# Linyou/Ced-NeRF

Hardware: AMD Instinct MI355X
Metric: samples_per_sec (render_image_test, 800x800 D-NeRF lego-shaped synthetic) (higher is better)
Workload: dtype f32 (MLP GEMMs: split-fp16 MFMA, 22-bit operands, fp32 accumulate)

## Files before the change

ced_nerf_amd/csrc/field.hip:

```cpp
#include <atomic>
#include <cstring>

#include "ced_common.hpp"
#include "field_args.hpp"
#include "field_kernel.hpp"

namespace ced {

std::atomic<int> g_field_spread_tiles{ 2 };
std::atomic<int> g_march_two_pass{ -1 };

int launch_field(const ced_field_desc *d, FieldArgs &A, void *stream)
{
    int rc = validate_hash(&d->hash, "field_forward");
    if (rc) return rc;
    if (d->hash.n_levels != 16) {
        set_error("field_forward: the fused kernel needs n_levels == 16 (got %d)", d->hash.n_levels);
        return CED_E_UNSUPPORTED;
    }
    CED_REQUIRE(d->time_mode >= 0 && d->time_mode <= 2, "field_forward: time_mode=%d", d->time_mode);
    CED_REQUIRE(d->packed_weights != nullptr, "field_forward: null packed_weights");
    CED_REQUIRE(d->mlp_precision >= CED_MLP_F32 && d->mlp_precision <= CED_MLP_F32_HEAD16X2, "field_forward: mlp_precision=%d",
                d->mlp_precision);
    CED_REQUIRE((int64_t)d->packed_floats == ced_packed_weight_words(d->use_div_offsets, d->time_mode, d->mlp_precision),
// ... 37 lines not shown
};

}

extern "C" int ced_set_option(const char *key, int value)
{
    CED_REQUIRE(key != nullptr, "set_option: null key");
    if (strcmp(key, "field_spread_tiles") == 0) {
        CED_REQUIRE(value >= 0 && value <= 2, "set_option: field_spread_tiles must be 0, 1 or 2 (field_tile_range)");
        ced::g_field_spread_tiles = value;
        return CED_OK;
    }
    if (strcmp(key, "march_two_pass") == 0) {
        CED_REQUIRE(value >= -1 && value <= 1, "set_option: march_two_pass must be -1 (automatic), 0 or 1");
        ced::g_march_two_pass = value;
        return CED_OK;
    }
    if (strcmp(key, "hash_grad_blocks") == 0) {
        CED_REQUIRE(value >= 0 && value <= (1 << 20), "set_option: hash_grad_blocks must be 0 (no cap) .. 2^20");
        ced::g_hash_grad_blocks = value;
        return CED_OK;
    }
    ced::set_error("set_option: unknown key '%s'", key);
    return CED_E_INVALID;
}

extern "C" int64_t ced_packed_weight_floats(int use_div_offsets, int time_mode)
{
    (void)use_div_offsets;
    return time_mode ? ced::Blob<true>::TOTAL : ced::Blob<false>::TOTAL;
// ... 81 lines not shown
```

ced_nerf_amd/csrc/field_args.hpp:

```cpp
#pragma once
#include <hip/hip_runtime.h>
#include <atomic>
#include <cstdint>

#include "../../include/cednerf_hip.h"
#include "ced_common.hpp"

namespace ced {

struct HashLevels {
    float scale[CED_MAX_LEVELS];
    uint32_t res[CED_MAX_LEVELS], offset[CED_MAX_LEVELS], size[CED_MAX_LEVELS], hashed[CED_MAX_LEVELS];
};

inline void fill_levels(HashLevels &lv, const ced_hash_desc &h)
{
    for (int l = 0; l < CED_MAX_LEVELS; ++l) {
        lv.scale[l] = h.scale[l]; lv.res[l] = h.res[l]; lv.offset[l] = h.offset[l];
        lv.size[l] = h.size[l]; lv.hashed[l] = h.hashed[l];
    }
}

inline int require_32bit_byte_offsets(const ced_hash_desc &h, const char *who)
{
// ... 14 lines not shown
            pairs = pairs && l + 1 < h.n_levels && (uint64_t)h.offset[l] + h.size[l] < h.total_entries;
        }
        const int dense = dense_modes ? (pairs ? 3 : 1) : 0;
        word |= (n_hashed == 0 ? dense : (n_hashed == 4 ? 2 : 0)) << (2 * i);
    }
    return word;
}

struct FieldArgs {
    int64_t n;
    const int64_t *n_dev;
    unsigned long long *stamp;
    const int64_t *base_dev;
    const float *pos, *t, *dir;
    const float *rays_o, *rays_d;
    const int64_t *ray_idx;
    const int32_t *ray_idx32;
    const float *t0, *t1, *timestamps;
    int rays_mode, t_per_ray, want_rgb;
    float *rgb, *sigma, *geo;
    float aabb[6];
    float moving_step;
    int use_div, time_mode;
    const void *weights;
    int table_dtype, temporal;
    int spread_tiles;
    int level_mode;
    int max_blocks;
    const void *table;
    HashLevels levels;
};

extern std::atomic<int> g_march_two_pass;
extern std::atomic<int> g_field_spread_tiles;
extern std::atomic<int> g_hash_grad_blocks;
constexpr int kFieldBlocksDefault = 256;

template <int NT, int THREADS, typename Kernel>
void launch_field_grid(Kernel kernel, const FieldArgs &A, void *stream)
{
    const int64_t n_tiles = (A.n + 16 * NT - 1) / (16 * NT);
    constexpr int waves = THREADS / 64;
    int64_t blocks = A.spread_tiles ? (n_tiles + 3) / 4 : (n_tiles + waves - 1) / waves;
    const int cap = A.max_blocks > 0 ? A.max_blocks : kFieldBlocksDefault;
    if (blocks > cap) blocks = cap;
    hipLaunchKernelGGL(kernel, dim3((unsigned)blocks), dim3(THREADS), 0, (hipStream_t)stream, A);
}

int validate_hash(const ced_hash_desc *h, const char *who);
// ... 6 lines not shown
```

ced_nerf_amd/csrc/field_device.hpp:

```cpp
#pragma once
#include <cstdint>

#include "ced_common.hpp"

namespace ced {

typedef float f4 __attribute__((ext_vector_type(4)));
typedef float f2 __attribute__((ext_vector_type(2)));

struct TileRange { int64_t first, end, stride; };
__device__ __forceinline__ bool field_tile_range(int mode, int64_t n_tiles, int waves, int wave, TileRange &r)
{
    const int64_t grid = gridDim.x, b = blockIdx.x;
    if (mode == 2 && (grid & 7) == 0) {
        const int64_t n_groups = (n_tiles + 3) >> 2, per_xcd = grid >> 3, region = (n_groups + 7) >> 3;
        const int64_t start = (b & 7) * region;
        const int64_t g_end = start + region < n_groups ? start + region : n_groups;
        if (start + (b >> 3) >= g_end) return false;
        r.first = (start + (int64_t)(wave >> 2) * per_xcd + (b >> 3)) * 4 + (wave & 3);
        r.end = 4 * g_end < n_tiles ? 4 * g_end : n_tiles;
        r.stride = (int64_t)(waves / 4) * per_xcd * 4;
        return true;
    }
    if ((mode ? b * 4 : b * waves) >= n_tiles) return false;
// ... 73 lines not shown
{
    typedef uint32_t u4 __attribute__((ext_vector_type(4)));
    const u4 a = *reinterpret_cast<const u4 *>(lt), b = *reinterpret_cast<const u4 *>(lt + 4);
    LevelConst L;
    L.scale = __uint_as_float(a[0]);
    L.sxb = a[1];
    L.syb = a[2];
    L.szb = a[3];
    L.offb = b[0];
    L.sizeb = b[1];
    L.maskb = b[2];
    L.hashed = b[3];
    return L;
}

template <bool F16, bool TEMPORAL, int MODE>
__device__ __forceinline__ void hash_level(const LevelConst &L, const void *__restrict__ table, const float (&x)[3],
                                           int k_lo, float t_frac, float &f0, float &f1)
{
    uint32_t g[3];
    float fr[3], om[3];
#pragma unroll
    for (int a = 0; a < 3; ++a) {
        const float p = x[a] * L.scale + 0.5f;
        g[a] = (uint32_t)p;
        fr[a] = __builtin_amdgcn_fractf(p);
        om[a] = 1.0f - fr[a];
    }
    constexpr uint32_t EB = EntryBytes<F16, TEMPORAL>::value;
    const uint32_t x0 = g[0] * EB;
    const uint32_t y0 = (MODE == 1 || MODE == 3) ? __umul24(g[1], L.syb) : g[1] * L.syb;
    const uint32_t z0 = (MODE == 1 || MODE == 3) ? __umul24(g[2], L.szb) : g[2] * L.szb;
    const uint32_t xs[2] = { x0, x0 + EB };
    const uint32_t ys[2] = { y0, y0 + L.syb };
    const uint32_t zs[2] = { z0, z0 + L.szb };
    const bool hashed = L.hashed != 0;
    uint32_t yz_x[4], yz_a[4];
#pragma unroll
    for (int q = 0; q < 4; ++q) {
        if constexpr (MODE != 1 && MODE != 3) yz_x[q] = ys[q & 1] ^ zs[q >> 1];
        if constexpr (MODE != 2) yz_a[q] = ys[q & 1] + zs[q >> 1];
    }
    const float wxy[4] = { om[0] * om[1], fr[0] * om[1], om[0] * fr[1], fr[0] * fr[1] };
    uint32_t off[8];
    float w[8];
#pragma unroll
    for (int c = 0; c < 8; ++c) {
        const int cx = c & 1, cy = (c >> 1) & 1, cz = (c >> 2) & 1;
        uint32_t hb = 0, db = 0;
        if constexpr (MODE != 1 && MODE != 3) hb = (xs[cx] ^ yz_x[cy + 2 * cz]) & L.maskb;
        if constexpr (MODE != 2) {
            const uint32_t dx = xs[cx] + yz_a[cy + 2 * cz];
            const uint32_t dw = dx - L.sizeb;
            db = dx < dw ? dx : dw;
        }
        const uint32_t idxb = (MODE == 1 || MODE == 3) ? db : (MODE == 2) ? hb : (hashed ? hb : db);
        off[c] = L.offb + idxb;
        w[c] = wxy[cx + 2 * cy] * (cz ? fr[2] : om[2]);
    }
    const char *tb = reinterpret_cast<const char *>(table);
    f2 v[8];
    if constexpr (!TEMPORAL) {
        if constexpr (MODE == 3) {
            constexpr uint32_t EBp = EntryBytes<F16, TEMPORAL>::value;
#pragma unroll
            for (int q = 0; q < 4; ++q) {
                if constexpr (!F16) {
                    const f4 pr = *reinterpret_cast<const f4 *>(tb + off[2 * q]);
                    v[2 * q] = f2{ pr[0], pr[1] };
                    v[2 * q + 1] = f2{ pr[2], pr[3] };
                    if (off[2 * q + 1] != off[2 * q] + EBp) v[2 * q + 1] = *reinterpret_cast<const f2 *>(tb + off[2 * q + 1]);
                } else {
                    typedef uint32_t u2v __attribute__((ext_vector_type(2)));
                    const u2v u = *reinterpret_cast<const u2v *>(tb + off[2 * q]);
                    uint32_t u1 = u[1];
                    if (off[2 * q + 1] != off[2 * q] + EBp) u1 = *reinterpret_cast<const uint32_t *>(tb + off[2 * q + 1]);
                    v[2 * q] = f2{ half_bits_to_float((uint16_t)(u[0] & 0xffffu)), half_bits_to_float((uint16_t)(u[0] >> 16)) };
                    v[2 * q + 1] = f2{ half_bits_to_float((uint16_t)(u1 & 0xffffu)), half_bits_to_float((uint16_t)(u1 >> 16)) };
                }
            }
        } else if constexpr (!F16) {
#pragma unroll
            for (int c = 0; c < 8; ++c) v[c] = *reinterpret_cast<const f2 *>(tb + off[c]);
        } else {
#pragma unroll
            for (int c = 0; c < 8; ++c) {
                const uint32_t u = *reinterpret_cast<const uint32_t *>(tb + off[c]);
                v[c] = f2{ half_bits_to_float((uint16_t)(u & 0xffffu)), half_bits_to_float((uint16_t)(u >> 16)) };
            }
        }
    } else {
        const float omt = 1.0f - t_frac;
        const f2 omt2 = { omt, omt }, tf2 = { t_frac, t_frac };
        const uint32_t kb = (uint32_t)k_lo * (F16 ? 4u : 8u);
        if constexpr (!F16) {
#pragma unroll
            for (int c = 0; c < 8; ++c) {
                const f4 pr = *reinterpret_cast<const f4 *>(tb + off[c] + kb);
                const f2 lo = { pr[0], pr[1] }, hi = { pr[2], pr[3] };
                v[c] = lo * omt2 + hi * tf2;
            }
        } else {
#pragma unroll
            for (int c = 0; c < 8; ++c) {
                typedef uint32_t u2t __attribute__((ext_vector_type(2)));
                const u2t pr = *reinterpret_cast<const u2t *>(tb + off[c] + kb);
                const uint32_t lo = pr[0], hi = pr[1];
                const f2 a = { half_bits_to_float((uint16_t)(lo & 0xffffu)), half_bits_to_float((uint16_t)(lo >> 16)) };
                const f2 b = { half_bits_to_float((uint16_t)(hi & 0xffffu)), half_bits_to_float((uint16_t)(hi >> 16)) };
                v[c] = a * omt2 + b * tf2;
            }
        }
    }
    f2 acc = { 0.0f, 0.0f };
#pragma unroll
    for (int c = 0; c < 8; ++c) acc = __builtin_elementwise_fma(f2{ w[c], w[c] }, v[c], acc);
    f0 = acc[0];
    f1 = acc[1];
}

template <bool F16, bool TEMPORAL, int MODE>
__device__ __forceinline__ void hash_level_dx(const LevelConst &L, const void *__restrict__ table, const float (&x)[3],
                                              int k_lo, float t_frac, float dscale, float &f0, float &f1, float (&d0)[3],
                                              float (&d1)[3])
{
    static_assert(MODE == 0 || MODE == 2, "hash_level_dx: mixed (0) or hashed (2) index form");
    uint32_t g[3];
// ... 59 lines not shown
    f2 gx = { 0.0f, 0.0f }, gy = { 0.0f, 0.0f }, gz = { 0.0f, 0.0f };
#pragma unroll
    for (int q = 0; q < 4; ++q) {
        const int lo = q & 1, hi = q >> 1;
        const float wyz = (lo ? fr[1] : om[1]) * (hi ? fr[2] : om[2]);
        const float wxz = (lo ? fr[0] : om[0]) * (hi ? fr[2] : om[2]);
        gx = __builtin_elementwise_fma(f2{ wyz, wyz }, v[1 + 2 * lo + 4 * hi] - v[2 * lo + 4 * hi], gx);
        gy = __builtin_elementwise_fma(f2{ wxz, wxz }, v[lo + 2 + 4 * hi] - v[lo + 4 * hi], gy);
        gz = __builtin_elementwise_fma(f2{ wxy[q], wxy[q] }, v[q + 4] - v[q], gz);
    }
    const float s = L.scale * dscale;
    d0[0] = gx[0] * s; d0[1] = gy[0] * s; d0[2] = gz[0] * s;
    d1[0] = gx[1] * s; d1[1] = gy[1] * s; d1[2] = gz[1] * s;
}

__device__ __forceinline__ void temporal_keyframe(float tq, int &k_lo, float &t_frac)
{
    float ts = tq * 3.0f;
    float fl = __builtin_floorf(ts);
    t_frac = ts - fl;
    fl = __builtin_fminf(fl, 2.0f);
    k_lo = (int)fl;
}

__device__ __forceinline__ float time_feature(int idx, int time_mode, float t, float mn)
{
    const float HALF_PI = 1.57079637050628662f;
    if (idx == 0) return t;
    if (idx > 8) return 0.0f;
    int k, ph;
// ... 14 lines not shown
```

ced_nerf_amd/csrc/field_half.hip:

```cpp
#include <cstring>

#include "ced_common.hpp"
#include "field_args.hpp"
#include "field_device.hpp"
#include "field_half_device.hpp"
#include "hash_device.hpp"

namespace ced {

template <bool TE, bool F16, bool TEMPORAL, bool SPLIT, int NT, int THREADS>
__global__ __launch_bounds__(THREADS) void field_half_kernel(FieldArgs A)
{
    constexpr int WAVES = THREADS / kWave;
    constexpr bool K32 = half_kernel_k32(TE, TEMPORAL, SPLIT, THREADS);
    static_assert(!K32 || (WAVES & (WAVES - 1)) == 0, "field_tile_seq needs a power-of-two wave count");
    constexpr int TILE = 16 * NT;
    using BL = HalfBlob<TE>;
    constexpr int PLANE = BL::FRAGS * kFragHalves;
    constexpr int WHALVES = PLANE * (SPLIT ? 2 : 1);
    __shared__ __attribute__((aligned(16))) _Float16 lds[WHALVES + 16 * CED_MAX_LEVELS];
    __shared__ int next_elem;
    const int tid = threadIdx.x;
    const int lane = tid & 63;
    const int wave = __builtin_amdgcn_readfirstlane(tid >> 6);
// ... 181 lines not shown
#pragma unroll
        for (int j = 0; j < NT; ++j) {
            const bool stored = 16 * j + c < in_tile;
            const int64_t s = tile_base + (16 * j + c);
            float sg = det_expf(D[j][0][3] - 1.0f);
            sg = sel[j] ? sg : 0.0f;
            if (g == 3 && stored) A.sigma[sbase + s] = sg;
            if (A.geo && stored) {
#pragma unroll
                for (int r = 0; r < 4; ++r)
                    if (4 * g + r < 15) A.geo[s * 15 + 4 * g + r] = D[j][0][r];
            }
        }

        if (A.want_rgb) {
#pragma unroll
            for (int j = 0; j < NT; ++j) {
                float dv[3];
#pragma unroll
                for (int a = 0; a < 3; ++a)
                    dv[a] = A.rays_mode ? A.rays_d[3 * ridx[j] + a] : A.dir[3 * (tile_base + sofs[j]) + a];
                const float nrm = __builtin_sqrtf((dv[0] * dv[0] + dv[1] * dv[1]) + dv[2] * dv[2]);
                const float comp = (g == 1) ? dv[1] : (g == 2) ? dv[2] : dv[0];
                const float u = (comp / nrm + 1.0f) / 2.0f;
                const float vv = u * 2.0f - 1.0f;
                const float coef = (g == 2) ? 0.48860251190291987f : -0.48860251190291987f;
                const float sh = (g == 0) ? 0.28209479177387814f : coef * vv;
                float hin[8];
                hin[0] = sh;
#pragma unroll
                for (int r = 0; r < 4; ++r) hin[1 + r] = __builtin_amdgcn_fmed3f(D[j][0][r], -kHalfMax, kHalfMax);
                hin[4] = (g == 3) ? 0.0f : hin[4];
                hin[5] = hin[6] = hin[7] = 0.0f;
                to_half8<SPLIT>(hin, Bh[j][0], Bl[j][0]);
            }
            mlp_layer_h<1, 4, NT, SPLIT>(whi + BL::H0 * kFragHalves, wlo + BL::H0 * kFragHalves, lane, Bh, Bl, D);
            to_operand_h<NT, SPLIT>(D, Bh, Bl);
            mlp_layer_h<2, 4, NT, SPLIT, K32>(whi + BL::H1 * kFragHalves, wlo + BL::H1 * kFragHalves, lane, Bh, Bl, D);
            to_operand_h<NT, SPLIT>(D, Bh, Bl);
            mlp_layer_h<2, 1, NT, SPLIT, K32>(whi + BL::H2 * kFragHalves, wlo + BL::H2 * kFragHalves, lane, Bh, Bl, D);
#pragma unroll
            for (int j = 0; j < NT; ++j) {
                const int64_t s = tile_base + (16 * j + c);
                const float o1 = 1.0f / (1.0f + det_expf(-D[j][0][0]));
// ... 142 lines not shown
```

ced_nerf_amd/csrc/field_kernel.hpp:

```cpp
#pragma once
#include "ced_common.hpp"
#include "field_args.hpp"
#include "field_device.hpp"
#include "field_half_device.hpp"
#include "hash_device.hpp"

namespace ced {

struct LayerShape { int nb; int ks; };
__host__ __device__ constexpr int ks4_of(int ks) { return (ks + 3) / 4; }
__host__ __device__ constexpr int layer_floats(int nb, int ks) { return nb * ks4_of(ks) * 256; }

__host__ __device__ constexpr int base_out_neuron(int p)
{
    const int g = p >> 2, r = p & 3;
    return r > 0 ? (4 * r + g - 3) : (g < 3 ? 13 + g : 0);
}

template <bool TE> struct Blob {
    static constexpr int KS_B0 = TE ? 11 : 8;
    static constexpr int M0 = 0;
    static constexpr int M1 = M0 + layer_floats(4, 8);
    static constexpr int M2 = M1 + layer_floats(4, 16);
    static constexpr int M3 = M2 + layer_floats(4, 16);
// ... 267 lines not shown
#pragma unroll
                for (int r = 0; r < 4; ++r) {
                    const int nidx = HEAD16 ? half_base_out_neuron(4 * g + r) : base_out_neuron(4 * g + r);
                    if (nidx >= 1) A.geo[s * 15 + nidx - 1] = D[j][0][r];
                }
            }
        }

        if constexpr (HEAD16) {
            if (A.want_rgb) {
                const _Float16 *const hw = reinterpret_cast<const _Float16 *>(lw + BL::H0);
                const _Float16 *const hwl = hw + BL::HEAD_FRAGS * kFragHalves;
                h8 Bh[NT][2], Bl[NT][2];
#pragma unroll
                for (int j = 0; j < NT; ++j) {
                    float dv[3];
#pragma unroll
                    for (int a = 0; a < 3; ++a)
                        dv[a] = A.rays_mode ? A.rays_d[3 * ridx[j] + a] : A.dir[3 * sidx[j] + a];
                    const float nrm = __builtin_sqrtf((dv[0] * dv[0] + dv[1] * dv[1]) + dv[2] * dv[2]);
                    const float comp = (g == 1) ? dv[1] : (g == 2) ? dv[2] : dv[0];
                    const float u = (comp / nrm + 1.0f) / 2.0f;
                    const float vv = u * 2.0f - 1.0f;
                    const float coef = (g == 2) ? 0.48860251190291987f : -0.48860251190291987f;
                    float hin[8];
                    hin[0] = (g == 0) ? 0.28209479177387814f : coef * vv;
#pragma unroll
                    for (int r = 0; r < 4; ++r) hin[1 + r] = __builtin_amdgcn_fmed3f(D[j][0][r], -kHalfMax, kHalfMax);
                    hin[4] = (g == 3) ? 0.0f : hin[4];
                    hin[5] = hin[6] = hin[7] = 0.0f;
                    to_half8<true>(hin, Bh[j][0], Bl[j][0]);
                }
                mlp_layer_h<1, 4, NT, true>(hw + BL::HF_H0 * kFragHalves, hwl + BL::HF_H0 * kFragHalves, lane, Bh, Bl, D);
                to_operand_h<NT, true>(D, Bh, Bl);
                mlp_layer_h<2, 4, NT, true>(hw + BL::HF_H1 * kFragHalves, hwl + BL::HF_H1 * kFragHalves, lane, Bh, Bl, D);
                to_operand_h<NT, true>(D, Bh, Bl);
                mlp_layer_h<2, 1, NT, true>(hw + BL::HF_H2 * kFragHalves, hwl + BL::HF_H2 * kFragHalves, lane, Bh, Bl, D);
#pragma unroll
                for (int j = 0; j < NT; ++j) {
                    const float o1 = 1.0f / (1.0f + det_expf(-D[j][0][0]));
                    int lane_now = (int)threadIdx.x;
                    asm volatile("" : "+v"(lane_now));
                    const int g_now = (lane_now >> 4) & 3;
                    const int64_t s_now = tile * TILE + 16 * j + (lane_now & 15);
                    if (g_now < 3 && s_now < n_eff) A.rgb[3 * (sbase + s_now) + g_now] = o1;
                }
            }
            continue;
        }

        if (A.want_rgb) {
#pragma unroll
            for (int j = 0; j < NT; ++j) {
                const float geo_tail = (g == 3) ? 0.0f : D[j][0][0];
                float dv[3];
#pragma unroll
                for (int a = 0; a < 3; ++a)
                    dv[a] = A.rays_mode ? A.rays_d[3 * ridx[j] + a] : A.dir[3 * sidx[j] + a];
                const float nrm = __builtin_sqrtf((dv[0] * dv[0] + dv[1] * dv[1]) + dv[2] * dv[2]);
                const float comp = (g == 1) ? dv[1] : (g == 2) ? dv[2] : dv[0];
                const float u = (comp / nrm + 1.0f) / 2.0f;
                const float vv = u * 2.0f - 1.0f;
                const float coef = (g == 2) ? 0.48860251190291987f : -0.48860251190291987f;
                B[j][0] = (g == 0) ? 0.28209479177387814f : coef * vv;
                B[j][1] = D[j][0][1];
                B[j][2] = D[j][0][2];
                B[j][3] = D[j][0][3];
                B[j][4] = geo_tail;
            }
            mlp_layer<5, 4, NT>(lw + BL::H0, lane, B, D);
            to_operand<4, true, NT>(D, B);
            mlp_layer<16, 4, NT>(lw + BL::H1, lane, B, D);
            to_operand<4, true, NT>(D, B);
            mlp_layer<16, 1, NT>(lw + BL::H2, lane, B, D);
#pragma unroll
            for (int j = 0; j < NT; ++j) {
                const int64_t s = tile * TILE + 16 * j + c;
                const float o1 = 1.0f / (1.0f + det_expf(-D[j][0][0]));
                int lane_now = (int)threadIdx.x;
// ... 12 lines not shown
```

ced_nerf_amd/csrc/frame.hip:

```cpp
#include <atomic>
#include <chrono>
#include <vector>

#include "ced_common.hpp"
#include "composite_core.hpp"
#include "field_args.hpp"
#include "march_accel.hpp"

#ifdef CED_MARCH_DIAG
__device__ unsigned long long g_march_diag[8][3];
__device__ __forceinline__ unsigned long long (*ced_diag_acc())[8][3]
{
    __shared__ unsigned long long acc[16][8][3];
    return acc;
}
__device__ __forceinline__ unsigned long long *ced_diag_state()
{
    __shared__ unsigned long long st[16][2];
    return &st[0][0];
}
__device__ void ced_diag_tick(int phase)
{
    const unsigned long long m = __ballot(1);
    const int wave = threadIdx.x >> 6;
// ... 129 lines not shown
    return block_base + wave_cnt[wave] + __builtin_popcountll(ballot & ((1ull << lane) - 1ull));
}

__global__ __launch_bounds__(256) void frame_times_kernel(int64_t n_rays, int rays_per_frame,
                                                          const float *__restrict__ frame_times, float *__restrict__ ts_ray)
{
    const int64_t r = (int64_t)blockIdx.x * blockDim.x + threadIdx.x;
    if (r < n_rays) ts_ray[r] = frame_times[r / rays_per_frame];
}

__global__ __launch_bounds__(256) void frame_prep_kernel(int64_t n_rays, const float *__restrict__ rays_o,
                                                         const float *__restrict__ rays_d, int m,
                                                         const float *__restrict__ aabbs, float near_plane,
                                                         float *__restrict__ t_sorted, uint8_t *__restrict__ t_indices,
                                                         uint8_t *__restrict__ hits, float *__restrict__ near_planes,
                                                         float *__restrict__ rgb,
                                                         float *__restrict__ opacity, float *__restrict__ depth)
{
    int64_t r = (int64_t)blockIdx.x * blockDim.x + threadIdx.x;
    if (r >= n_rays) return;
    const float o[3] = { rays_o[3 * r], rays_o[3 * r + 1], rays_o[3 * r + 2] };
    const float inv_d[3] = { 1.0f / rays_d[3 * r], 1.0f / rays_d[3 * r + 1], 1.0f / rays_d[3 * r + 2] };
    float ev[2 * kMaxGrids];
    int id[2 * kMaxGrids];
    for (int a = 0; a < m; ++a) {
        float t0 = __builtin_inff(), t1 = __builtin_inff();
        bool hit = slab_test(o, inv_d, aabbs + 6 * a, t0, t1);
        if (!hit) { t0 = __builtin_inff(); t1 = __builtin_inff(); }
        hits[r * m + a] = hit ? 1 : 0;
        ev[a] = t0; id[a] = a;
        ev[m + a] = t1; id[m + a] = m + a;
    }
    if (m > 1) {
        for (int i = 1; i < 2 * m; ++i) {
            float v = ev[i];
            int k = id[i], j = i - 1;
            while (j >= 0 && ev[j] > v) { ev[j + 1] = ev[j]; id[j + 1] = id[j]; --j; }
            ev[j + 1] = v; id[j + 1] = k;
        }
    }
    for (int i = 0; i < 2 * m; ++i) {
        t_sorted[r * 2 * m + i] = ev[i];
        t_indices[r * 2 * m + i] = (uint8_t)id[i];
    }
    near_planes[r] = near_plane;
    rgb[3 * r] = 0.0f; rgb[3 * r + 1] = 0.0f; rgb[3 * r + 2] = 0.0f;
    opacity[r] = 0.0f;
    depth[r] = 0.0f;
}

__global__ __launch_bounds__(256) void frame_prep_single_kernel(int64_t n_rays, float near_plane, float *__restrict__ near_planes,
                                                                float *__restrict__ rgb, float *__restrict__ opacity,
                                                                float *__restrict__ depth)
{
    int64_t r = (int64_t)blockIdx.x * blockDim.x + threadIdx.x;
    if (r >= n_rays) return;
    near_planes[r] = near_plane;
    rgb[3 * r] = 0.0f; rgb[3 * r + 1] = 0.0f; rgb[3 * r + 2] = 0.0f;
    opacity[r] = 0.0f;
    depth[r] = 0.0f;
}

struct ScheduleArgs {
    IterPlan *plans;
    int it, n_frames, rays_per_frame, min_samples, max_samples;
    long long *host;
    long long seq;
    const int32_t *local_rays;
    const int64_t *xcounts;
    int64_t global_rays;
    long long *host_iter;
// ... 319 lines not shown
{
    const int f = threadIdx.x;
    if (f >= n_frames) return;
    const unsigned long long nx = __hip_atomic_load(&plan->next[f], __ATOMIC_RELAXED, __HIP_MEMORY_SCOPE_AGENT);
    const bool finished = plan->last[f] || plan->gcount[f] == 0 || plan->count[f] == 0;
    row[f] = finished ? 0 : (int64_t)(nx & 0xffffffffull);
}

struct ImageState {
    int32_t *cursor;
    float *acc_all;
    float *acc_kept;
    int32_t *kept;
};

__global__ __launch_bounds__(256) void image_prep_kernel(int64_t n_rays, ImageState st, float *__restrict__ rgb,
                                                         float *__restrict__ opacity, float *__restrict__ depth)
{
    int64_t r = (int64_t)blockIdx.x * blockDim.x + threadIdx.x;
    if (r >= n_rays) return;
    st.cursor[r] = 0; st.acc_all[r] = 0.0f; st.acc_kept[r] = 0.0f; st.kept[r] = 0;
    if (rgb) {
        rgb[3 * r] = 0.0f; rgb[3 * r + 1] = 0.0f; rgb[3 * r + 2] = 0.0f;
        opacity[r] = 0.0f;
        depth[r] = 0.0f;
    }
}

__device__ __forceinline__ int64_t ray_count(const int64_t *__restrict__ packed_all, int64_t r, int64_t n_all)
{
    const int64_t start = packed_all[2 * r], cnt = packed_all[2 * r + 1];
    return (start < 0 || cnt < 0 || start + cnt > n_all) ? 0 : cnt;
}

__global__ __launch_bounds__(kMarchThreads) void image_chunk_kernel(
    IterPlan *__restrict__ plan, int64_t n_all, const int32_t *__restrict__ alive, const int64_t *__restrict__ packed_all,
    const float *__restrict__ t0_all, const float *__restrict__ t1_all, const int32_t *__restrict__ cursor,
// ... 220 lines not shown
    {
        T *p = (T *)(base + off);
        off = (off + count * sizeof(T) + 255) & ~(size_t)255;
        return p;
    }
};

struct FrameWorkspace {
    float *t_sorted; uint8_t *t_indices; uint8_t *hits; float *near; int32_t *packed;
    int32_t *alive_a, *alive_b;
    IterPlan *plans;
    float *lattice;
    float *ts_ray;
    float *t0, *t1; int32_t *ridx; float *sigma, *rgbs;
    uint8_t *accel;
    size_t bytes;
};

static inline int min_samples_of(float cone_angle) { return cone_angle == 0.0f ? 1 : 4; }
static inline int max_iterations(int max_samples, int min_samples) { return (max_samples + min_samples - 1) / min_samples; }

static inline int64_t sample_capacity(int n_frames, int64_t rays_per_frame, int min_samples, int64_t global_rays)
{
    int64_t per = rays_per_frame * min_samples;
    if (global_rays > rays_per_frame) {
        const int64_t worst = rays_per_frame * 64 < global_rays ? rays_per_frame * 64 : global_rays;
        if (worst > per) per = worst;
    }
    return per * n_frames;
}
// ... 7 lines not shown
    w.hits = c.take<uint8_t>((size_t)n * m);
    w.near = c.take<float>((size_t)n);
    w.packed = c.take<int32_t>((size_t)n * 2);
    w.alive_a = c.take<int32_t>((size_t)n);
    w.alive_b = c.take<int32_t>((size_t)n);
    w.plans = c.take<IterPlan>((size_t)max_iters + 2);
    w.lattice = c.take<float>(256);
    w.ts_ray = c.take<float>(per_ray_times ? (size_t)n : 0);
    w.t0 = c.take<float>((size_t)cap);
    w.t1 = c.take<float>((size_t)cap);
    w.ridx = c.take<int32_t>((size_t)cap);
    w.sigma = c.take<float>((size_t)cap);
    w.rgbs = c.take<float>((size_t)cap * 3);
    const int64_t nbk = (res + kBrick - 1) / kBrick;
    w.accel = c.take<uint8_t>((size_t)(2 * m * nbk * nbk * nbk));
    w.bytes = c.off;
    return w;
}

static std::atomic<long long> g_publish_seq{ 0 };

#if defined(__HIP_DEVICE_COMPILE__)
#define CED_CPU_PAUSE()
#else
#define CED_CPU_PAUSE() __builtin_ia32_pause()
#endif

static int wait_published(volatile long long *flag, long long seq, hipStream_t stream, const char *who)
{
    const auto t_start = std::chrono::steady_clock::now();
// ... 92 lines not shown
    CED_REQUIRE(cap < (1ll << 31) - 64, "%s: too many samples per iteration for 32-bit sample indices", who);
    const int max_iters = max_iterations(max_samples, min_samples);
    FrameWorkspace W = carve(workspace, n_rays, n_grids, cap, max_iters, res, frame_times != nullptr);
    CED_REQUIRE((int64_t)W.bytes <= workspace_bytes, "%s: workspace too small (%lld < %lld bytes)", who,
                (long long)workspace_bytes, (long long)W.bytes);
    if (xch) {
        CED_REQUIRE(xch->reduce && xch->counts && xch->global_rays_per_frame >= rays_per_frame &&
                        xch->global_rays_per_frame < (1ll << 31),
                    "%s: bad ced_shard_exchange (reduce / counts NULL, or global_rays_per_frame < rays_per_frame)", who);
        CED_REQUIRE(!field_stream_ || field_stream_ == stream_, "%s: a sharded call takes no separate field stream", who);
    }
    long long *const host_iter = xch ? (long long *)host_stats + kHostIterWord : nullptr;
    const dim3 blk(256), grd((unsigned)((n_rays + 255) / 256));

    if (n_grids == 1)
        hipLaunchKernelGGL(frame_prep_single_kernel, grd, blk, 0, stream, n_rays, near_plane, W.near, rgb, opacity, depth);
    else
        hipLaunchKernelGGL(frame_prep_kernel, grd, blk, 0, stream, n_rays, rays_o, rays_d, (int)n_grids, aabbs, near_plane,
                           W.t_sorted, W.t_indices, W.hits, W.near, rgb, opacity, depth);
    if (frame_times)
        hipLaunchKernelGGL(frame_times_kernel, grd, blk, 0, stream, n_rays, (int)rays_per_frame, frame_times, W.ts_ray);
    const int nb = (res + kBrick - 1) / kBrick;
    AccelSpec acc;
    if (accel) {
        acc = accel_view(accel, n_grids, res, true);
    } else {
        int rc = build_brick_accel(binaries, n_grids, res, W.accel, W.accel + (size_t)n_grids * nb * nb * nb, stream);
        if (rc) return rc;
        acc = AccelSpec{ W.accel, nb, nullptr };
    }
    volatile long long *pub = (volatile long long *)host_stats;
    std::vector<long long> plan_seq((size_t)max_iters + 1);
    plan_seq[0] = ++g_publish_seq;
    const bool use_lattice = cone_angle == 0.0f && step_size > 0.0f && near_plane >= 0.0f;
// ... 42 lines not shown
            }
        } else if (it == 0) {
            if (n_grids == 1) hipLaunchKernelGGL((march_frame_kernel<true, false, true>), dim3((unsigned)mgrid), mblk, 0, stream, M, plan);
            else hipLaunchKernelGGL((march_frame_kernel<false, false, true>), dim3((unsigned)mgrid), mblk, 0, stream, M, plan);
        } else {
            if (n_grids == 1) hipLaunchKernelGGL((march_frame_kernel<true, false, false>), dim3((unsigned)mgrid), mblk, 0, stream, M, plan);
            else hipLaunchKernelGGL((march_frame_kernel<false, false, false>), dim3((unsigned)mgrid), mblk, 0, stream, M, plan);
        }
        rc = check_launch("render_image_test (march)");
        if (rc) return rc;

        FieldArgs F{};
        F.n = cap;
        F.n_dev = &plan->total_samples;
        F.rays_o = rays_o; F.rays_d = rays_d; F.ray_idx32 = W.ridx;
        F.t0 = W.t0; F.t1 = W.t1;
        F.timestamps = frame_times ? W.ts_ray : timestamps;
        F.rays_mode = 1; F.t_per_ray = (frame_times || t_per_ray) ? 1 : 0; F.want_rgb = 1;
        F.rgb = W.rgbs; F.sigma = W.sigma; F.geo = nullptr;
        if (trace && trace->field_stamps && it < trace->capacity)
            F.stamp = reinterpret_cast<unsigned long long *>(trace->field_stamps) + 2 * it;
        if (split) {
            (void)hipEventRecord(ev_to_field[dev], stream);
            (void)hipStreamWaitEvent(fstream, ev_to_field[dev], 0);
        }
        if (trace && it < trace->capacity && trace->field_begin)
            (void)hipEventRecord((hipEvent_t)trace->field_begin[it], fstream);
        rc = launch_field(field, F, (void *)fstream);
        if (rc) return rc;
        if (trace && it < trace->capacity && trace->field_end)
// ... 52 lines not shown
            if (trace->iter_n_samples) trace->iter_n_samples[k] = max_limit;
            if (trace->iter_samples) trace->iter_samples[k] = samples_it;
        }
    }
    if (trace) trace->n_iters = n_iters;
    if (total_samples_out)
        for (int f = 0; f < n_frames; ++f) total_samples_out[f] = total[f];
    return CED_OK;
}

struct ImageWorkspace {
    ImageState st;
    int32_t *packed, *alive_a, *alive_b;
    IterPlan *plans;
    float *t0, *t1; int32_t *ridx; float *sigma, *rgbs, *w, *tr, *al; int32_t *rank;
    size_t bytes;
};

constexpr int kImageMaxIters = 1024;

static ImageWorkspace carve_image(void *base, int64_t n, int64_t cap)
{
    ImageWorkspace w{};
    Carver c{ (char *)base };
    w.st.cursor = c.take<int32_t>((size_t)n);
    w.st.acc_all = c.take<float>((size_t)n);
    w.st.acc_kept = c.take<float>((size_t)n);
    w.packed = c.take<int32_t>((size_t)n * 2);
    w.alive_a = c.take<int32_t>((size_t)n);
    w.alive_b = c.take<int32_t>((size_t)n);
    w.plans = c.take<IterPlan>((size_t)kImageMaxIters + 2);
    w.t0 = c.take<float>((size_t)cap);
    w.t1 = c.take<float>((size_t)cap);
    w.ridx = c.take<int32_t>((size_t)cap);
    w.sigma = c.take<float>((size_t)cap);
    w.rgbs = c.take<float>((size_t)cap * 3);
    w.w = c.take<float>((size_t)cap);
    w.tr = c.take<float>((size_t)cap);
    w.al = c.take<float>((size_t)cap);
    w.rank = c.take<int32_t>((size_t)cap);
    w.bytes = c.off;
    return w;
}

static inline int64_t image_capacity(int64_t n_rays, int64_t n_all) { return n_all + 64; }

static int render_image_impl(const ced_field_desc *field, int64_t n_rays, const float *rays_o, const float *rays_d,
                             int64_t n_all, const int64_t *packed_all, const float *t0_all, const float *t1_all,
                             float early_stop_eps, float alpha_thre, const float *timestamps, int32_t t_per_ray,
                             const float *bkgd, float *rgb, float *opacity, float *depth, int32_t *kept, void *workspace,
                             int64_t workspace_bytes, int64_t *host_stats, int64_t *stats_out, void *field_stream_,
                             void *stream_)
{
    const char *who = "render_image";
    hipStream_t stream = (hipStream_t)stream_;
// ... 2 lines not shown
    CED_REQUIRE(field != nullptr, "%s: null field descriptor", who);
    CED_REQUIRE(n_rays >= 0 && n_all >= 0, "%s: bad sizes", who);
    CED_REQUIRE(n_rays < (1ll << 31) / 4 && n_all < (1ll << 31) - 128, "%s: too many rays / samples for 32-bit indices", who);
    if (stats_out) { stats_out[0] = 0; stats_out[1] = 0; stats_out[2] = 0; }
    if (n_rays == 0) return CED_OK;
    const bool full = rgb != nullptr;
    CED_REQUIRE(rays_o && rays_d && packed_all && (n_all == 0 || (t0_all && t1_all)) && timestamps && kept && workspace &&
                    host_stats && (!full || (opacity && depth)),
                "%s: null pointer", who);
    const int64_t cap = image_capacity(n_rays, n_all);
    ImageWorkspace W = carve_image(workspace, n_rays, cap);
    W.st.kept = kept;
    CED_REQUIRE((int64_t)W.bytes <= workspace_bytes, "%s: workspace too small (%lld < %lld bytes)", who,
                (long long)workspace_bytes, (long long)W.bytes);
    const dim3 blk(256), grd((unsigned)((n_rays + 255) / 256));
    hipLaunchKernelGGL(image_prep_kernel, grd, blk, 0, stream, n_rays, W.st, rgb, opacity, depth);
    volatile long long *pub = (volatile long long *)host_stats;
    std::vector<long long> plan_seq((size_t)kImageMaxIters + 1);
    plan_seq[0] = ++g_publish_seq;
    const int big = 1 << 30;
    const int min_chunk = full ? 4 : 8;
    hipLaunchKernelGGL(frame_init_kernel, dim3(1), dim3(64), 0, stream,
                       ScheduleArgs{ W.plans, -1, 1, (int)n_rays, min_chunk, big, (long long *)host_stats, plan_seq[0] }, (float *)nullptr,
                       (unsigned long long *)nullptr, 0);
    int rc = check_launch("render_image (prep)");
    if (rc) return rc;
    long long alive_bound = n_rays;
    int it = 0;
    for (; it < kImageMaxIters; ++it) {
        bool stop = false;
        rc = run_ahead(pub, nullptr, plan_seq, it, stream, who, stop, alive_bound);
        if (rc) return rc;
        if (stop) break;
        IterPlan *plan = W.plans + it;
        const int32_t *cur_list = it == 0 ? nullptr : ((it & 1) ? W.alive_a : W.alive_b);
        int32_t *next_list = (it & 1) ? W.alive_b : W.alive_a;
        int64_t mgrid = (alive_bound + kMarchThreads - 1) / kMarchThreads;
        if (mgrid > 8192) mgrid = 8192;
        if (mgrid < 1) mgrid = 1;
        hipLaunchKernelGGL(image_chunk_kernel, dim3((unsigned)mgrid), dim3(kMarchThreads), 0, stream, plan, n_all, cur_list,
                           packed_all, t0_all, t1_all, W.st.cursor, W.t0, W.t1, W.ridx, W.packed);
        FieldArgs F{};
        F.n = n_rays * (int64_t)min_chunk;
        F.n_dev = &plan->total_samples;
        F.base_dev = &plan->sample_base;
        F.rays_o = rays_o; F.rays_d = rays_d; F.ray_idx32 = W.ridx;
        F.t0 = W.t0; F.t1 = W.t1;
        F.timestamps = timestamps;
        F.rays_mode = 1; F.t_per_ray = t_per_ray ? 1 : 0; F.want_rgb = full ? 1 : 0;
        F.rgb = full ? W.rgbs : nullptr; F.sigma = W.sigma; F.geo = nullptr;
        rc = launch_field(field, F, (void *)stream);
        if (rc) return rc;
        int64_t cgrid = (alive_bound + kCompositeThreads - 1) / kCompositeThreads;
        if (cgrid > 4096) cgrid = 4096;
        if (cgrid < 1) cgrid = 1;
        plan_seq[it + 1] = ++g_publish_seq;
        if (full)
            hipLaunchKernelGGL(image_composite_kernel<true>, dim3((unsigned)cgrid), dim3(kCompositeThreads), 0, stream, plan,
                               cur_list, next_list, W.packed, packed_all, W.t0, W.t1, W.sigma, W.rgbs, W.st, W.w, W.tr, W.al,
                               W.rank, rgb, opacity, depth, early_stop_eps, alpha_thre, n_all);
        else
// ... 202 lines not shown
```

Measured before the change: 4.471 billion.

## Precompute per-ray SH inputs and add dense-level fast path for corner offsets

Adds a per-ray spherical-harmonics precompute in the prep kernels, stored in workspace, so the field kernel's color head loads one float per sample instead of reading three direction components and doing a sqrt and divide each time. Separately, the hash-level lookup gains a wave-uniform check: when no corner index in the wave wraps past the level size, dense levels compute offsets with plain adds and use adjacent-pair loads without the per-pair adjacency test. The cost is extra workspace (three floats per ray), an extra global load, and a ballot per level.

```diff
diff --git a/ced_nerf_amd/csrc/field.hip b/ced_nerf_amd/csrc/field.hip
--- a/ced_nerf_amd/csrc/field.hip
+++ b/ced_nerf_amd/csrc/field.hip
@@ -8,6 +8,7 @@
 namespace ced {
 
 std::atomic<int> g_field_spread_tiles{ 2 };
+std::atomic<int> g_frame_sh_per_ray{ 1 };
 std::atomic<int> g_march_two_pass{ -1 };
 
 int launch_field(const ced_field_desc *d, FieldArgs &A, void *stream)
@@ -75,6 +76,11 @@
     if (strcmp(key, "march_two_pass") == 0) {
         CED_REQUIRE(value >= -1 && value <= 1, "set_option: march_two_pass must be -1 (automatic), 0 or 1");
         ced::g_march_two_pass = value;
+        return CED_OK;
+    }
+    if (strcmp(key, "frame_sh_per_ray") == 0) {
+        CED_REQUIRE(value == 0 || value == 1, "set_option: frame_sh_per_ray must be 0 or 1");
+        ced::g_frame_sh_per_ray = value;
         return CED_OK;
     }
     if (strcmp(key, "hash_grad_blocks") == 0) {
diff --git a/ced_nerf_amd/csrc/field_args.hpp b/ced_nerf_amd/csrc/field_args.hpp
--- a/ced_nerf_amd/csrc/field_args.hpp
+++ b/ced_nerf_amd/csrc/field_args.hpp
@@ -52,6 +52,7 @@
     const int64_t *base_dev;
     const float *pos, *t, *dir;
     const float *rays_o, *rays_d;
+    const float *sh_ray;
     const int64_t *ray_idx;
     const int32_t *ray_idx32;
     const float *t0, *t1, *timestamps;
@@ -71,6 +72,7 @@
 
 extern std::atomic<int> g_march_two_pass;
 extern std::atomic<int> g_field_spread_tiles;
+extern std::atomic<int> g_frame_sh_per_ray;
 extern std::atomic<int> g_hash_grad_blocks;
 constexpr int kFieldBlocksDefault = 256;
 
diff --git a/ced_nerf_amd/csrc/field_device.hpp b/ced_nerf_amd/csrc/field_device.hpp
--- a/ced_nerf_amd/csrc/field_device.hpp
+++ b/ced_nerf_amd/csrc/field_device.hpp
@@ -111,6 +111,66 @@
     return L;
 }
 
+template <bool F16, bool TEMPORAL, bool PAIRS, bool ADJACENT>
+__device__ __forceinline__ void load_corners(const char *__restrict__ tb, const uint32_t (&off)[8], int k_lo, float t_frac,
+                                             f2 (&v)[8])
+{
+    if constexpr (!TEMPORAL) {
+        if constexpr (PAIRS) {
+            constexpr uint32_t EBp = EntryBytes<F16, TEMPORAL>::value;
+#pragma unroll
+            for (int q = 0; q < 4; ++q) {
+                if constexpr (!F16) {
+                    const f4 pr = *reinterpret_cast<const f4 *>(tb + off[2 * q]);
+                    v[2 * q] = f2{ pr[0], pr[1] };
+                    v[2 * q + 1] = f2{ pr[2], pr[3] };
+                    if constexpr (!ADJACENT)
+                        if (off[2 * q + 1] != off[2 * q] + EBp) v[2 * q + 1] = *reinterpret_cast<const f2 *>(tb + off[2 * q + 1]);
+                } else {
+                    typedef uint32_t u2v __attribute__((ext_vector_type(2)));
+                    const u2v u = *reinterpret_cast<const u2v *>(tb + off[2 * q]);
+                    uint32_t u1 = u[1];
+                    if constexpr (!ADJACENT)
+                        if (off[2 * q + 1] != off[2 * q] + EBp) u1 = *reinterpret_cast<const uint32_t *>(tb + off[2 * q + 1]);
+                    v[2 * q] = f2{ half_bits_to_float((uint16_t)(u[0] & 0xffffu)), half_bits_to_float((uint16_t)(u[0] >> 16)) };
+                    v[2 * q + 1] = f2{ half_bits_to_float((uint16_t)(u1 & 0xffffu)), half_bits_to_float((uint16_t)(u1 >> 16)) };
+                }
+            }
+        } else if constexpr (!F16) {
+#pragma unroll
+            for (int c = 0; c < 8; ++c) v[c] = *reinterpret_cast<const f2 *>(tb + off[c]);
+        } else {
+#pragma unroll
+            for (int c = 0; c < 8; ++c) {
+                const uint32_t u = *reinterpret_cast<const uint32_t *>(tb + off[c]);
+                v[c] = f2{ half_bits_to_float((uint16_t)(u & 0xffffu)), half_bits_to_float((uint16_t)(u >> 16)) };
+            }
+        }
+    } else {
+        const float omt = 1.0f - t_frac;
+        const f2 omt2 = { omt, omt }, tf2 = { t_frac, t_frac };
+        const uint32_t kb = (uint32_t)k_lo * (F16 ? 4u : 8u);
+        if constexpr (!F16) {
+#pragma unroll
+            for (int c = 0; c < 8; ++c) {
+                const f4 pr = *reinterpret_cast<const f4 *>(tb + off[c] + kb);
+                const f2 lo = { pr[0], pr[1] }, hi = { pr[2], pr[3] };
+                v[c] = lo * omt2 + hi * tf2;
+            }
+        } else {
+#pragma unroll
+            for (int c = 0; c < 8; ++c) {
+                typedef uint32_t u2t __attribute__((ext_vector_type(2)));
+                const u2t pr = *reinterpret_cast<const u2t *>(tb + off[c] + kb);
+                const uint32_t lo = pr[0], hi = pr[1];
+                const f2 a = { half_bits_to_float((uint16_t)(lo & 0xffffu)), half_bits_to_float((uint16_t)(lo >> 16)) };
+                const f2 b = { half_bits_to_float((uint16_t)(hi & 0xffffu)), half_bits_to_float((uint16_t)(hi >> 16)) };
+                v[c] = a * omt2 + b * tf2;
+            }
+        }
+    }
+}
+
 template <bool F16, bool TEMPORAL, int MODE>
 __device__ __forceinline__ void hash_level(const LevelConst &L, const void *__restrict__ table, const float (&x)[3],
                                            int k_lo, float t_frac, float &f0, float &f1)
@@ -139,75 +199,43 @@
         if constexpr (MODE != 2) yz_a[q] = ys[q & 1] + zs[q >> 1];
     }
     const float wxy[4] = { om[0] * om[1], fr[0] * om[1], om[0] * fr[1], fr[0] * fr[1] };
+    float w[8];
+#pragma unroll
+    for (int c = 0; c < 8; ++c) w[c] = wxy[c & 3] * ((c >> 2) ? fr[2] : om[2]);
+    const char *tb = reinterpret_cast<const char *>(table);
     uint32_t off[8];
-    float w[8];
-#pragma unroll
-    for (int c = 0; c < 8; ++c) {
-        const int cx = c & 1, cy = (c >> 1) & 1, cz = (c >> 2) & 1;
-        uint32_t hb = 0, db = 0;
-        if constexpr (MODE != 1 && MODE != 3) hb = (xs[cx] ^ yz_x[cy + 2 * cz]) & L.maskb;
-        if constexpr (MODE != 2) {
-            const uint32_t dx = xs[cx] + yz_a[cy + 2 * cz];
-            const uint32_t dw = dx - L.sizeb;
-            db = dx < dw ? dx : dw;
-        }
-        const uint32_t idxb = (MODE == 1 || MODE == 3) ? db : (MODE == 2) ? hb : (hashed ? hb : db);
-        off[c] = L.offb + idxb;
-        w[c] = wxy[cx + 2 * cy] * (cz ? fr[2] : om[2]);
-    }
-    const char *tb = reinterpret_cast<const char *>(table);
     f2 v[8];
-    if constexpr (!TEMPORAL) {
-        if constexpr (MODE == 3) {
-            constexpr uint32_t EBp = EntryBytes<F16, TEMPORAL>::value;
-#pragma unroll
-            for (int q = 0; q < 4; ++q) {
-                if constexpr (!F16) {
-                    const f4 pr = *reinterpret_cast<const f4 *>(tb + off[2 * q]);
-                    v[2 * q] = f2{ pr[0], pr[1] };
-                    v[2 * q + 1] = f2{ pr[2], pr[3] };
-                    if (off[2 * q + 1] != off[2 * q] + EBp) v[2 * q + 1] = *reinterpret_cast<const f2 *>(tb + off[2 * q + 1]);
-                } else {
-                    typedef uint32_t u2v __attribute__((ext_vector_type(2)));
-                    const u2v u = *reinterpret_cast<const u2v *>(tb + off[2 * q]);
-                    uint32_t u1 = u[1];
-                    if (off[2 * q + 1] != off[2 * q] + EBp) u1 = *reinterpret_cast<const uint32_t *>(tb + off[2 * q + 1]);
-                    v[2 * q] = f2{ half_bits_to_float((uint16_t)(u[0] & 0xffffu)), half_bits_to_float((uint16_t)(u[0] >> 16)) };
-                    v[2 * q + 1] = f2{ half_bits_to_float((uint16_t)(u1 & 0xffffu)), half_bits_to_float((uint16_t)(u1 >> 16)) };
-                }
-            }
-        } else if constexpr (!F16) {
-#pragma unroll
-            for (int c = 0; c < 8; ++c) v[c] = *reinterpret_cast<const f2 *>(tb + off[c]);
+    if constexpr (MODE == 1 || MODE == 3) {
+        if (__ballot(xs[1] + yz_a[3] >= L.sizeb) == 0ull) {
+            uint32_t yz_o[4];
+#pragma unroll
+            for (int q = 0; q < 4; ++q) yz_o[q] = yz_a[q] + L.offb;
+#pragma unroll
+            for (int c = 0; c < 8; ++c) off[c] = xs[c & 1] + yz_o[c >> 1];
+            load_corners<F16, TEMPORAL, MODE == 3, true>(tb, off, k_lo, t_frac, v);
         } else {
 #pragma unroll
             for (int c = 0; c < 8; ++c) {
-                const uint32_t u = *reinterpret_cast<const uint32_t *>(tb + off[c]);
-                v[c] = f2{ half_bits_to_float((uint16_t)(u & 0xffffu)), half_bits_to_float((uint16_t)(u >> 16)) };
-            }
+                const uint32_t dx = xs[c & 1] + yz_a[c >> 1];
+                const uint32_t dw = dx - L.sizeb;
+                off[c] = L.offb + (dx < dw ? dx : dw);
+            }
+            load_corners<F16, TEMPORAL, MODE == 3, false>(tb, off, k_lo, t_frac, v);
         }
     } else {
-        const float omt = 1.0f - t_frac;
-        const f2 omt2 = { omt, omt }, tf2 = { t_frac, t_frac };
-        const uint32_t kb = (uint32_t)k_lo * (F16 ? 4u : 8u);
-        if constexpr (!F16) {
-#pragma unroll
-            for (int c = 0; c < 8; ++c) {
-                const f4 pr = *reinterpret_cast<const f4 *>(tb + off[c] + kb);
-                const f2 lo = { pr[0], pr[1] }, hi = { pr[2], pr[3] };
-                v[c] = lo * omt2 + hi * tf2;
-            }
-        } else {
-#pragma unroll
-            for (int c = 0; c < 8; ++c) {
-                typedef uint32_t u2t __attribute__((ext_vector_type(2)));
-                const u2t pr = *reinterpret_cast<const u2t *>(tb + off[c] + kb);
-                const uint32_t lo = pr[0], hi = pr[1];
-                const f2 a = { half_bits_to_float((uint16_t)(lo & 0xffffu)), half_bits_to_float((uint16_t)(lo >> 16)) };
-                const f2 b = { half_bits_to_float((uint16_t)(hi & 0xffffu)), half_bits_to_float((uint16_t)(hi >> 16)) };
-                v[c] = a * omt2 + b * tf2;
-            }
-        }
+#pragma unroll
+        for (int c = 0; c < 8; ++c) {
+            const uint32_t hb = (xs[c & 1] ^ yz_x[c >> 1]) & L.maskb;
+            uint32_t idxb = hb;
+            if constexpr (MODE == 0) {
+                const uint32_t dx = xs[c & 1] + yz_a[c >> 1];
+                const uint32_t dw = dx - L.sizeb;
+                const uint32_t db = dx < dw ? dx : dw;
+                idxb = hashed ? hb : db;
+            }
+            off[c] = L.offb + idxb;
+        }
+        load_corners<F16, TEMPORAL, false, false>(tb, off, k_lo, t_frac, v);
     }
     f2 acc = { 0.0f, 0.0f };
 #pragma unroll
@@ -297,6 +325,27 @@
     d1[0] = gx[1] * s; d1[1] = gy[1] * s; d1[2] = gz[1] * s;
 }
 
+__device__ __forceinline__ float sh_head_input(const float (&dv)[3], int g)
+{
+    const float nrm = __builtin_sqrtf((dv[0] * dv[0] + dv[1] * dv[1]) + dv[2] * dv[2]);
+    const float comp = (g == 1) ? dv[1] : (g == 2) ? dv[2] : dv[0];
+    const float u = (comp / nrm + 1.0f) / 2.0f;
+    const float vv = u * 2.0f - 1.0f;
+    const float coef = (g == 2) ? 0.48860251190291987f : -0.48860251190291987f;
+    return (g == 0) ? 0.28209479177387814f : coef * vv;
+}
+__device__ __forceinline__ void sh_ray_store(const float *__restrict__ rays_d, int64_t r, float *__restrict__ sh_ray)
+{
+    const float dv[3] = { rays_d[3 * r], rays_d[3 * r + 1], rays_d[3 * r + 2] };
+#pragma unroll
+    for (int g = 1; g < 4; ++g) sh_ray[3 * r + g - 1] = sh_head_input(dv, g);
+}
+__device__ __forceinline__ float sh_ray_load(const float *__restrict__ sh_ray, int64_t r, int g)
+{
+    const float v = sh_ray[3 * r + (g ? g - 1 : 0)];
+    return (g == 0) ? 0.28209479177387814f : v;
+}
+
 __device__ __forceinline__ void temporal_keyframe(float tq, int &k_lo, float &t_frac)
 {
     float ts = tq * 3.0f;
diff --git a/ced_nerf_amd/csrc/field_half.hip b/ced_nerf_amd/csrc/field_half.hip
--- a/ced_nerf_amd/csrc/field_half.hip
+++ b/ced_nerf_amd/csrc/field_half.hip
@@ -219,20 +219,19 @@
         }
 
         if (A.want_rgb) {
+            const bool sh_per_ray = A.rays_mode && A.sh_ray;
 #pragma unroll
             for (int j = 0; j < NT; ++j) {
-                float dv[3];
-#pragma unroll
-                for (int a = 0; a < 3; ++a)
-                    dv[a] = A.rays_mode ? A.rays_d[3 * ridx[j] + a] : A.dir[3 * (tile_base + sofs[j]) + a];
-                const float nrm = __builtin_sqrtf((dv[0] * dv[0] + dv[1] * dv[1]) + dv[2] * dv[2]);
-                const float comp = (g == 1) ? dv[1] : (g == 2) ? dv[2] : dv[0];
-                const float u = (comp / nrm + 1.0f) / 2.0f;
-                const float vv = u * 2.0f - 1.0f;
-                const float coef = (g == 2) ? 0.48860251190291987f : -0.48860251190291987f;
-                const float sh = (g == 0) ? 0.28209479177387814f : coef * vv;
                 float hin[8];
-                hin[0] = sh;
+                if (sh_per_ray) {
+                    hin[0] = sh_ray_load(A.sh_ray, ridx[j], g);
+                } else {
+                    float dv[3];
+#pragma unroll
+                    for (int a = 0; a < 3; ++a)
+                        dv[a] = A.rays_mode ? A.rays_d[3 * ridx[j] + a] : A.dir[3 * (tile_base + sofs[j]) + a];
+                    hin[0] = sh_head_input(dv, g);
+                }
 #pragma unroll
                 for (int r = 0; r < 4; ++r) hin[1 + r] = __builtin_amdgcn_fmed3f(D[j][0][r], -kHalfMax, kHalfMax);
                 hin[4] = (g == 3) ? 0.0f : hin[4];
diff --git a/ced_nerf_amd/csrc/field_kernel.hpp b/ced_nerf_amd/csrc/field_kernel.hpp
--- a/ced_nerf_amd/csrc/field_kernel.hpp
+++ b/ced_nerf_amd/csrc/field_kernel.hpp
@@ -305,17 +305,16 @@
                 h8 Bh[NT][2], Bl[NT][2];
 #pragma unroll
                 for (int j = 0; j < NT; ++j) {
-                    float dv[3];
-#pragma unroll
-                    for (int a = 0; a < 3; ++a)
-                        dv[a] = A.rays_mode ? A.rays_d[3 * ridx[j] + a] : A.dir[3 * sidx[j] + a];
-                    const float nrm = __builtin_sqrtf((dv[0] * dv[0] + dv[1] * dv[1]) + dv[2] * dv[2]);
-                    const float comp = (g == 1) ? dv[1] : (g == 2) ? dv[2] : dv[0];
-                    const float u = (comp / nrm + 1.0f) / 2.0f;
-                    const float vv = u * 2.0f - 1.0f;
-                    const float coef = (g == 2) ? 0.48860251190291987f : -0.48860251190291987f;
                     float hin[8];
-                    hin[0] = (g == 0) ? 0.28209479177387814f : coef * vv;
+                    if (A.rays_mode && A.sh_ray) {
+                        hin[0] = sh_ray_load(A.sh_ray, ridx[j], g);
+                    } else {
+                        float dv[3];
+#pragma unroll
+                        for (int a = 0; a < 3; ++a)
+                            dv[a] = A.rays_mode ? A.rays_d[3 * ridx[j] + a] : A.dir[3 * sidx[j] + a];
+                        hin[0] = sh_head_input(dv, g);
+                    }
 #pragma unroll
                     for (int r = 0; r < 4; ++r) hin[1 + r] = __builtin_amdgcn_fmed3f(D[j][0][r], -kHalfMax, kHalfMax);
                     hin[4] = (g == 3) ? 0.0f : hin[4];
@@ -344,16 +343,15 @@
 #pragma unroll
             for (int j = 0; j < NT; ++j) {
                 const float geo_tail = (g == 3) ? 0.0f : D[j][0][0];
-                float dv[3];
-#pragma unroll
-                for (int a = 0; a < 3; ++a)
-                    dv[a] = A.rays_mode ? A.rays_d[3 * ridx[j] + a] : A.dir[3 * sidx[j] + a];
-                const float nrm = __builtin_sqrtf((dv[0] * dv[0] + dv[1] * dv[1]) + dv[2] * dv[2]);
-                const float comp = (g == 1) ? dv[1] : (g == 2) ? dv[2] : dv[0];
-                const float u = (comp / nrm + 1.0f) / 2.0f;
-                const float vv = u * 2.0f - 1.0f;
-                const float coef = (g == 2) ? 0.48860251190291987f : -0.48860251190291987f;
-                B[j][0] = (g == 0) ? 0.28209479177387814f : coef * vv;
+                if (A.rays_mode && A.sh_ray) {
+                    B[j][0] = sh_ray_load(A.sh_ray, ridx[j], g);
+                } else {
+                    float dv[3];
+#pragma unroll
+                    for (int a = 0; a < 3; ++a)
+                        dv[a] = A.rays_mode ? A.rays_d[3 * ridx[j] + a] : A.dir[3 * sidx[j] + a];
+                    B[j][0] = sh_head_input(dv, g);
+                }
                 B[j][1] = D[j][0][1];
                 B[j][2] = D[j][0][2];
                 B[j][3] = D[j][0][3];
diff --git a/ced_nerf_amd/csrc/frame.hip b/ced_nerf_amd/csrc/frame.hip
--- a/ced_nerf_amd/csrc/frame.hip
+++ b/ced_nerf_amd/csrc/frame.hip
@@ -5,6 +5,7 @@
 #include "ced_common.hpp"
 #include "composite_core.hpp"
 #include "field_args.hpp"
+#include "field_device.hpp"
 #include "march_accel.hpp"
 
 #ifdef CED_MARCH_DIAG
@@ -167,11 +168,12 @@
                                                          const float *__restrict__ aabbs, float near_plane,
                                                          float *__restrict__ t_sorted, uint8_t *__restrict__ t_indices,
                                                          uint8_t *__restrict__ hits, float *__restrict__ near_planes,
-                                                         float *__restrict__ rgb,
+                                                         float *__restrict__ sh_ray, float *__restrict__ rgb,
                                                          float *__restrict__ opacity, float *__restrict__ depth)
 {
     int64_t r = (int64_t)blockIdx.x * blockDim.x + threadIdx.x;
     if (r >= n_rays) return;
+    sh_ray_store(rays_d, r, sh_ray);
     const float o[3] = { rays_o[3 * r], rays_o[3 * r + 1], rays_o[3 * r + 2] };
     const float inv_d[3] = { 1.0f / rays_d[3 * r], 1.0f / rays_d[3 * r + 1], 1.0f / rays_d[3 * r + 2] };
     float ev[2 * kMaxGrids];
@@ -202,12 +204,14 @@
     depth[r] = 0.0f;
 }
 
-__global__ __launch_bounds__(256) void frame_prep_single_kernel(int64_t n_rays, float near_plane, float *__restrict__ near_planes,
-                                                                float *__restrict__ rgb, float *__restrict__ opacity,
-                                                                float *__restrict__ depth)
+__global__ __launch_bounds__(256) void frame_prep_single_kernel(int64_t n_rays, const float *__restrict__ rays_d,
+                                                                float near_plane, float *__restrict__ near_planes,
+                                                                float *__restrict__ sh_ray, float *__restrict__ rgb,
+                                                                float *__restrict__ opacity, float *__restrict__ depth)
 {
     int64_t r = (int64_t)blockIdx.x * blockDim.x + threadIdx.x;
     if (r >= n_rays) return;
+    sh_ray_store(rays_d, r, sh_ray);
     near_planes[r] = near_plane;
     rgb[3 * r] = 0.0f; rgb[3 * r + 1] = 0.0f; rgb[3 * r + 2] = 0.0f;
     opacity[r] = 0.0f;
@@ -557,13 +561,15 @@
     int32_t *kept;
 };
 
-__global__ __launch_bounds__(256) void image_prep_kernel(int64_t n_rays, ImageState st, float *__restrict__ rgb,
+__global__ __launch_bounds__(256) void image_prep_kernel(int64_t n_rays, ImageState st, const float *__restrict__ rays_d,
+                                                         float *__restrict__ sh_ray, float *__restrict__ rgb,
                                                          float *__restrict__ opacity, float *__restrict__ depth)
 {
     int64_t r = (int64_t)blockIdx.x * blockDim.x + threadIdx.x;
     if (r >= n_rays) return;
     st.cursor[r] = 0; st.acc_all[r] = 0.0f; st.acc_kept[r] = 0.0f; st.kept[r] = 0;
     if (rgb) {
+        sh_ray_store(rays_d, r, sh_ray);
         rgb[3 * r] = 0.0f; rgb[3 * r + 1] = 0.0f; rgb[3 * r + 2] = 0.0f;
         opacity[r] = 0.0f;
         depth[r] = 0.0f;
@@ -814,6 +820,7 @@
     float *ts_ray;
     float *t0, *t1; int32_t *ridx; float *sigma, *rgbs;
     uint8_t *accel;
+    float *sh_ray;
     size_t bytes;
 };
 
@@ -851,6 +858,7 @@
     w.rgbs = c.take<float>((size_t)cap * 3);
     const int64_t nbk = (res + kBrick - 1) / kBrick;
     w.accel = c.take<uint8_t>((size_t)(2 * m * nbk * nbk * nbk));
+    w.sh_ray = c.take<float>((size_t)n * 3);
     w.bytes = c.off;
     return w;
 }
@@ -973,10 +981,11 @@
     const dim3 blk(256), grd((unsigned)((n_rays + 255) / 256));
 
     if (n_grids == 1)
-        hipLaunchKernelGGL(frame_prep_single_kernel, grd, blk, 0, stream, n_rays, near_plane, W.near, rgb, opacity, depth);
+        hipLaunchKernelGGL(frame_prep_single_kernel, grd, blk, 0, stream, n_rays, rays_d, near_plane, W.near, W.sh_ray, rgb,
+                           opacity, depth);
     else
         hipLaunchKernelGGL(frame_prep_kernel, grd, blk, 0, stream, n_rays, rays_o, rays_d, (int)n_grids, aabbs, near_plane,
-                           W.t_sorted, W.t_indices, W.hits, W.near, rgb, opacity, depth);
+                           W.t_sorted, W.t_indices, W.hits, W.near, W.sh_ray, rgb, opacity, depth);
     if (frame_times)
         hipLaunchKernelGGL(frame_times_kernel, grd, blk, 0, stream, n_rays, (int)rays_per_frame, frame_times, W.ts_ray);
     const int nb = (res + kBrick - 1) / kBrick;
@@ -1049,6 +1058,7 @@
         F.n = cap;
         F.n_dev = &plan->total_samples;
         F.rays_o = rays_o; F.rays_d = rays_d; F.ray_idx32 = W.ridx;
+        F.sh_ray = g_frame_sh_per_ray ? W.sh_ray : nullptr;
         F.t0 = W.t0; F.t1 = W.t1;
         F.timestamps = frame_times ? W.ts_ray : timestamps;
         F.rays_mode = 1; F.t_per_ray = (frame_times || t_per_ray) ? 1 : 0; F.want_rgb = 1;
@@ -1131,6 +1141,7 @@
     int32_t *packed, *alive_a, *alive_b;
     IterPlan *plans;
     float *t0, *t1; int32_t *ridx; float *sigma, *rgbs, *w, *tr, *al; int32_t *rank;
+    float *sh_ray;
     size_t bytes;
 };
 
@@ -1156,6 +1167,7 @@
     w.tr = c.take<float>((size_t)cap);
     w.al = c.take<float>((size_t)cap);
     w.rank = c.take<int32_t>((size_t)cap);
+    w.sh_ray = c.take<float>((size_t)n * 3);
     w.bytes = c.off;
     return w;
 }
@@ -1188,7 +1200,7 @@
     CED_REQUIRE((int64_t)W.bytes <= workspace_bytes, "%s: workspace too small (%lld < %lld bytes)", who,
                 (long long)workspace_bytes, (long long)W.bytes);
     const dim3 blk(256), grd((unsigned)((n_rays + 255) / 256));
-    hipLaunchKernelGGL(image_prep_kernel, grd, blk, 0, stream, n_rays, W.st, rgb, opacity, depth);
+    hipLaunchKernelGGL(image_prep_kernel, grd, blk, 0, stream, n_rays, W.st, rays_d, W.sh_ray, rgb, opacity, depth);
     volatile long long *pub = (volatile long long *)host_stats;
     std::vector<long long> plan_seq((size_t)kImageMaxIters + 1);
     plan_seq[0] = ++g_publish_seq;
@@ -1219,6 +1231,7 @@
         F.n_dev = &plan->total_samples;
         F.base_dev = &plan->sample_base;
         F.rays_o = rays_o; F.rays_d = rays_d; F.ray_idx32 = W.ridx;
+        F.sh_ray = (full && g_frame_sh_per_ray) ? W.sh_ray : nullptr;
         F.t0 = W.t0; F.t1 = W.t1;
         F.timestamps = timestamps;
         F.rays_mode = 1; F.t_per_ray = t_per_ray ? 1 : 0; F.want_rgb = full ? 1 : 0;
```

New measurement: 4.553 billion (median of 6 runs). 1.02x the previous value.
